# crabml/crabml

Measured on AMD Instinct MI355X. Metric: decode tokens/sec (batch-1 greedy), Llama-3-8B shape Q4_0, higher is better.
Workload: dtype q4_0 x q8_0 -> i32 dot, f32 accumulate

## Files before the change

### crabml_amd/csrc/fused.hip

```cpp
#include <chrono>
#include <thread>
#include <cmath>

#include "fused_common.hpp"
#include "fused_attention.hpp"
#include "fused_ffn.hpp"
#include "sampler.hpp"
#include "prefill_rows.hpp"
#include "lazy.hpp"


#include <dlfcn.h>

using namespace crabml_hip;

struct crabml_hip_tp_comm {
  crabml_hip_device* dev = nullptr;
  void* nccl = nullptr;
  int nranks = 1, rank = 0;
  bool p2p = false;
  bool connected = false;
  unsigned long long* inbox = nullptr;
  bool via_ipc[8] = {false};
  size_t inbox_bytes = 0;
  unsigned cap = 0;
  bool finegrained = false;
  void* peer[8] = {nullptr};
  int* fault = nullptr;
  unsigned host_epoch = 0;
  unsigned sessions = 0;
};
namespace {
struct NcclId {
  char b[128];
};
struct Rccl {
  typedef NcclId IdT;
  void* lib = nullptr;
  int (*GetUniqueId)(void*) = nullptr;
// ... 81 lines not shown
  float* h = nullptr;
  float* logits = nullptr;
  float* host_logits = nullptr;
  unsigned out_seq = 0;
  unsigned lazy_serial = 0;
  bool ext_kv = false;
  const crabml_hip_buf* ext_kc0 = nullptr;
  float* tmp = nullptr;
  char* act_dim = nullptr;
  char* act_attn = nullptr;
  char* act_hid = nullptr;
  float* rope = nullptr;
  int* state = nullptr;
  unsigned long long* slots = nullptr;
  unsigned long long* a8gran = nullptr;
  unsigned long long* h8gran = nullptr;
  bool q8k_producers = false;
  unsigned tp_salt = 0;
  bool tp_dry = false;
  bool k_norm_in = false;
  bool kfused = false;
  bool generic = false;
  bool ord = false;
  uint32_t qt = 0, out_qt = 0;
  float* xn = nullptr;
  bool norm_epi = false;
  bool defer_norm = false;
  float* rsums = nullptr;
  bool norm_epi_k = false;
  unsigned* out_tokens = nullptr;
  int out_cap = 0;
  float* am_val = nullptr;
  int* am_idx = nullptr;
  bool split_vocab = false;
  int vocab_l = 0, vocab_off = 0;
  int* am_best = nullptr;
  bool sampling = false;
  float* sm_bmax = nullptr;
  unsigned short* sm_keys = nullptr;
  unsigned* sm_hist = nullptr;
  float* sm_par = nullptr;
  float* sm_coins = nullptr;
  hipGraph_t sgraph[3] = {nullptr, nullptr, nullptr};
  hipGraphExec_t sexec[3] = {nullptr, nullptr, nullptr};
  size_t kv_len = 0;
  hipGraph_t graph[3] = {nullptr, nullptr, nullptr};
  hipGraphExec_t exec[3] = {nullptr, nullptr, nullptr};
  bool use_graph = false;
  bool capturing = false;
  int attn_variant = 0;
  size_t flash_ticket_until = 0;
  bool attn_long_ok = false;
  bool exact_long_ok = false;
  size_t attn_long_from = 0;
  bool pv_split = false;
  bool attn_flash = false;
  bool flash_ticket = false;
  bool attn_flash_rows = false;
  int flash_S = 0;
  int flash_min_rows = FLASH_MIN_ROWS;
  float* flash_part = nullptr;
  unsigned* flash_tick = nullptr;
  int gu_rows = 0;
  int attn_s_rows = 0;
  size_t attn_s_lds = 0;
  float* scores_g = nullptr;
// ... 299 lines not shown
  if (prof) prof_begin(dev, &ar, CRABML_HIP_F32, 7, 0.0);
  if (c->attn_s_rows > 0)
    launch_k(st, AR, attn_s_kernel(hd), dim3(n_heads + spare), dim3(256), c->attn_s_lds, (const float*)c->qbuf, (const unsigned short*)c->kc[l],
             (const unsigned short*)c->vc[l], pos_d, (const unsigned short*)dev->exp_table, c->attn, xq, xd, xisum, n_heads, n_kv, hd, seq_cap,
             c->attn_s_rows, pf, (k8 ? 2 : c->qt == CRABML_HIP_Q8_1 ? 1 : 0) | sbit, (long long*)nullptr, k8 ? *k8 : AttnQ8K{});
  else
    with_const_else<0, 1>(c->cfg.use_f16_kv_cache != 0, [&](auto kv16) {
      launch_k(st, AR, k_attn<decltype(kv16)::value != 0>, dim3(n_heads + spare), dim3(256), attn_lds, (const float*)c->qbuf, (const void*)c->kc[l],
               (const void*)c->vc[l], pos_d, (const unsigned short*)dev->exp_table, c->attn, xq, xd, xisum, n_heads, n_kv, hd,
               seq_cap, pf, (c->qt == CRABML_HIP_Q8_1 ? 1 : 0) | sbit, (long long*)nullptr);
    });
  if (prof) prof_end(dev, &ar);
}

int enqueue_classifier_and_sampler(crabml_hip_llama* c, const void* cls_act, bool prof) {
  crabml_hip_device* dev = c->dev;
  hipStream_t st = dev->stream;
  const auto& g = c->cfg;
  const int dim = (int)g.embedding_dim;
  int *token_d = c->state, *pos_d = c->state + 1, *step_d = c->state + 2;
  float* out = c->logits + c->vocab_off;
  crabml_hip_device::ProfRec pr{};
  const uint32_t ot = c->output->dtype;
  if (prof)
    CH_TRY(prof_begin(dev, &pr, ot, 5, (double)c->vocab_l * (double)(dim / block_elems(ot)) * (double)block_bytes(ot) + 4.0 * dim + 4.0 * c->vocab_l));
  if (dev->strict_order)
    CH_TRY(launch_gemv_strict(dev, c->output, (size_t)c->vocab_l, dim, cls_act, 1, out));
  else
    CH_TRY(launch_gemv(dev, c->output, (size_t)c->vocab_l, dim, cls_act, 1, out, prof ? &pr : nullptr));
  if (prof) CH_TRY(prof_end(dev, &pr));
  if (c->ext_kv) {
    if (c->host_logits != nullptr) {
      const int n = c->vocab_l;
      k_logits_to_host<<<64, 256, 0, st>>>((const f32x4*)out, (f32x4*)c->host_logits, n / 4, out, c->host_logits, n);
      k_host_flag<<<1, 1, 0, st>>>((unsigned*)(c->host_logits + c->cfg.vocab_size), (const int*)(c->state + 7), c->state + 5);
    }
    CH_HIP(dev, hipGetLastError());
    return 0;
  }
  if (c->sampling) {
    const int n = c->vocab_l;
    const SampleStep ss{c->sm_par, c->sm_coins, token_d, pos_d, step_d, c->state + 4, c->out_tokens, c->out_cap, c->state + 5};
    k_sample_max<<<SAMPLE_BLOCKS, 256, 0, st>>>(out, n, c->sm_par, c->sm_bmax);
    k_sample_keys<<<SAMPLE_BLOCKS, 256, 0, st>>>(out, n, c->sm_par, c->sm_bmax, SAMPLE_BLOCKS, (const unsigned short*)dev->exp_table,
                                                 c->sm_keys, c->sm_hist);
    if (dev->strict_order)
      k_sample_pick<true><<<1, SAMPLE_PICK_THREADS, 0, st>>>(c->sm_keys, n, c->sm_hist, ss);
    else
      k_sample_pick<false><<<1, SAMPLE_PICK_THREADS, 0, st>>>(c->sm_keys, n, c->sm_hist, ss);
    CH_HIP(dev, hipGetLastError());
    return 0;
  }
  k_argmax_partial<<<ARGMAX_BLOCKS, 256, 0, st>>>(out, c->vocab_l, c->am_val, c->am_idx, c->vocab_off);
  if (c->split_vocab && c->comm && c->comm->p2p)
    k_argmax_step_tp<<<1, 64, 0, st>>>(c->am_val, c->am_idx, ARGMAX_BLOCKS, token_d, pos_d, step_d, c->out_tokens, c->out_cap, c->state + 4,
                                       tp_view(c, true), n_segments(c));
  else
    k_argmax_step<<<1, 64, 0, st>>>(c->am_val, c->am_idx, ARGMAX_BLOCKS, token_d, pos_d, step_d, c->out_tokens, c->out_cap, c->state + 4,
                                    c->split_vocab ? c->am_best : (int*)nullptr);
  CH_HIP(dev, hipGetLastError());
  return 0;
}

static QkvEpiB qwen2_epi(const crabml_hip_llama* c, const QkvEpi& e, int l) {
  return QkvEpiB{e, (const float*)c->bq[l]->ptr, (const float*)c->bk[l]->ptr, (const float*)c->bv[l]->ptr};
}
template <class E>
struct QkvArchOf {
  static constexpr int value = QKV_LLAMA;
};
template <>
struct QkvArchOf<QkvEpiB> {
  static constexpr int value = QKV_QWEN2;
};
template <>
struct QkvArchOf<QkvEpiN> {
  static constexpr int value = QKV_GEMMA;
};
template <class F>
void with_qkv_epi(const crabml_hip_llama* c, const QkvEpi& e, int l, F&& f) {
  if (c->qwen2)
    f(qwen2_epi(c, e, l));
  else if (c->gemma)
    f(QkvEpiN{e});
  else
    f(e);
}
// ... 26 lines not shown
  const int L = (int)g.n_layers;
  constexpr bool Q81 = FMT == CRABML_HIP_Q4_1;
  const uint32_t qt = c->qt;
  ActPtrs ad = act_ptrs(c->act_dim, dim, qt), aa = act_ptrs(c->act_attn, dim_l, qt), ah = act_ptrs(c->act_hid, hidden_l, qt);
  const bool prof = dev->prof_on && !c->use_graph && !c->capturing;
  const double blk_b = (double)block_bytes(c->wtype) / 32.0;
  auto P0 = [&](crabml_hip_device::ProfRec* r, uint32_t stage, double rows, double k) {
    return prof ? prof_begin(dev, r, c->wtype, stage, rows * k * blk_b + 4.0 * k + 4.0 * rows) : 0;
  };
  auto P1 = [&](crabml_hip_device::ProfRec* r) { return prof ? prof_end(dev, r) : 0; };
  crabml_hip_device::ProfRec pr{};
  crabml_hip_device::ProfRec* R = prof ? &pr : nullptr;
  const bool do_pf = !(g.flags & CRABML_HIP_LLAMA_NO_PREFETCH);
  auto plan = [&](const crabml_hip_buf* a, const crabml_hip_buf* b, const crabml_hip_buf* cc) {
    PrefetchPlan pf{};
    const crabml_hip_buf* v[3] = {a, b, cc};
    for (int i = 0; i < 3; i++) {
      pf.p[i] = do_pf && v[i] ? v[i]->ptr : nullptr;
      pf.n[i] = do_pf && v[i] ? (v[i]->wl.total / 16) * 16 : 0;
    }
    pf.sink = c->state + 3;
    return pf;
  };
  const int spare = do_pf ? (dev->n_cu > 1 ? dev->n_cu - 1 : 0) : 0;
  const size_t norm_lds = norm_lds_bytes(dim);
  auto norm_quant = [&](const float* wn, float eps, bool add_pending, const PrefetchPlan& pf) {
    crabml_hip_device::ProfRec nr{};
    if (prof) prof_begin(dev, &nr, CRABML_HIP_F32, 6, 8.0 * dim);
    const float* addv = add_pending ? c->partial : nullptr;
    with_const_else<4, 12>(norm_nit(dim), [&](auto nit) {
      launch_k(st, prof ? &nr : nullptr, k_norm_quant<decltype(nit)::value, Q81>, dim3(1 + spare), dim3(1024), norm_lds, c->x, addv, wn, dim, eps, ad.q,
               ad.d, ad.isum, pf, c->ord ? 0 : 1);
    });
    if (prof) prof_end(dev, &nr);
  };
  const bool norm_epi = c->norm_epi;
  static const int qkv_upfront = test_hook_off("CRABML_HIP_QKV_UPFRONT") ? 0 : 1;
  const bool defer_wo = c->defer_norm && !Q81;
  const bool defer_down = c->defer_norm && !Q81;
  auto gemv_out = [&](const crabml_hip_buf* w, const ActPtrs& a, int k, uint32_t stage, const float* wnext, float eps_next, bool defer = false,
                      const float* xin = nullptr) -> int {
    CH_TRY(P0(&pr, stage, dim, k));
    float* dst = tp ? c->partial : c->x;
    if (norm_epi) {
      NormGather ng{c->slots, c->slots + dim / 16, c->state + 4, c->state + 5, n_segments(c), seg, c->rsums};
      const int split = chunk_split(g.flags, k, dim, dev->n_cu);
      c->tap.note(seg / 2, stage == 2 ? CRABML_HIP_PLAN_SPLIT_WO : CRABML_HIP_PLAN_SPLIT_DOWN, split);
      const TpP2P tpv = tp_view(c, tp);
      auto nq = [&](auto form, size_t lds, const float* rhs, auto tparg) {
        with_const_else<2, 1>(split, [&](auto s) {
          launch_k(st, R, nq_kernel<FMT, decltype(s)::value>(form), dim3(dim / 32 * split), dim3(1024), lds, planes_of(w), act_view<FMT>(a), rhs, c->x,
                   wnext, eps_next, ad.q, ad.d, ad.isum, ng, k / 32, Planes6{nullptr, 0}, tparg);
        });
      };
      if (xin != nullptr && !Q81) {
        if constexpr (!Q81) {
          if (tpv.n > 1)
            nq(NqForm<1, true>{}, q8_0_lds_bytes(k / 32), xin, tpv);
          else
            nq(NqForm<1>{}, q8_0_lds_bytes(k / 32), xin, NoTp{});
        }
      } else if (tpv.n > 1) {
        nq(NqForm<0, true>{}, 0, nullptr, tpv);
      } else if (c->ord) {
        static const int pipe_mode = test_hook_int("CRABML_HIP_ORD_PIPE", -1);
        const int pipe = pipe_mode >= 0 ? pipe_mode : FMT == CRABML_HIP_Q8_0 ? 2 : 1;
// ... 12 lines not shown
    } else if (c->ord) {
      launch_k(st, R, k_gemv_res_ord<FMT>, dim3((dim + 7) / 8), dim3(256), ord_terms_lds_bytes(k / 32), planes_of(w), act_view<FMT>(a), c->x, dim, k / 32);
    } else if (tp) {
      launch_k(st, R, k_gemv_res<FMT, 1, false>, dim3((dim + 1) / 2), dim3(128), 0, planes_of(w), act_view<FMT>(a), dst, dim, k / 32);
    } else {
      launch_k(st, R, k_gemv_res<FMT, 1, true>, dim3((dim + 1) / 2), dim3(128), 0, planes_of(w), act_view<FMT>(a), dst, dim, k / 32);
    }
    CH_TRY(P1(&pr));
    return 0;
  };

  const size_t ad_bytes = act_layout(qt, (size_t)dim).total, rs_bytes = c->rsums ? (size_t)(dim / 32) * 4 : 0;
  TapRec& tap = c->tap;
  auto TAP = [&](bool on, int f, const void* src, size_t bytes) -> int { return on ? tap.copy(c, f, src, bytes) : 0; };
  if (seg == 2 * L) {
    const void* cls_act = c->act_dim;
    if (c->out_qt != qt) {
      const float* addv = tp && !norm_epi ? c->partial : nullptr;
      launch_norm_f32(st, c->x, addv, (const float*)c->rms_final->ptr, dim, g.rms_norm_eps, c->xn, c->ord ? 0 : 1);
      if (c->out_qt == CRABML_HIP_F32) {
        cls_act = c->xn;
      } else {
        launch_quantize_act(st, c->out_qt, c->xn, (size_t)dim, c->act_dim);
      }
    } else if (!norm_epi) {
      norm_quant((const float*)c->rms_final->ptr, g.rms_norm_eps, tp, plan(nullptr, nullptr, nullptr));
      CH_TRY(TAP(tap.layer == L - 1, CRABML_HIP_TAP_DOWN_ACT, c->act_dim, ad_bytes));
    }
    CH_TRY(TAP(true, CRABML_HIP_TAP_CLS_ACT, cls_act, c->out_qt == CRABML_HIP_F32 ? (size_t)dim * 4 : act_layout(c->out_qt, (size_t)dim).total));
    return enqueue_classifier_and_sampler(c, cls_act, prof);
  }
  const int l = seg / 2;
  if ((seg & 1) == 0) {
    if (l == 0) launch_embed(c);
    if (!norm_epi || l == 0)
      norm_quant((const float*)c->rms_att[l]->ptr, g.rms_norm_eps, tp && l > 0, plan(c->wq[l], c->wk[l], c->wv[l]));
    const bool tl = tap.layer == l;
    if (!norm_epi || l == 0) tap.note(l, CRABML_HIP_PLAN_NORM_NIT, norm_nit(dim));
    CH_TRY(TAP(!norm_epi && l > 0 && tap.layer == l - 1, CRABML_HIP_TAP_DOWN_ACT, c->act_dim, ad_bytes));
    CH_TRY(TAP(tl, CRABML_HIP_TAP_QKV_IN_X, c->x, (size_t)dim * 4));
    CH_TRY(TAP(tl, CRABML_HIP_TAP_QKV_IN_ACT, c->act_dim, ad_bytes));
    CH_TRY(TAP(tl, CRABML_HIP_TAP_QKV_IN_RSUMS, c->rsums, rs_bytes));
    const QkvEpi e = decode_qkv_epi(c, l);
    const int total_rows = dim_l + 2 * kv_dim_l;
    CH_TRY(P0(&pr, 1, total_rows, dim));
    const RmsTail rtq{c->rsums, dim / 32, 1.0f / (float)dim, g.rms_norm_eps};
    const bool deferq = defer_down && l > 0;
    const int upfront = deferq ? qkv_upfront : (qkv_upfront && total_rows / 2 <= 4 * dev->n_cu) ? 1 : 0;
    if (!c->ord) {
      const int nu = dim / 32 * BlockFmt<FMT>::UNITS;
      tap.note(l, CRABML_HIP_PLAN_QKV_LOADER, deferq ? (upfront && nu == 128 ? 4 : 3) : (upfront && nu % 128 == 0 ? 2 : 1));
    }
    with_qkv_epi(c, e, l, [&](auto ep) {
      constexpr int A = QkvArchOf<decltype(ep)>::value;
      if (c->ord)
        launch_k(st, R, k_qkv_ord<FMT, A>, dim3((total_rows / 2 + 3) / 4), dim3(256), ord_terms_lds_bytes(dim / 32), planes_of(c->wq[l]),
                 planes_of(c->wk[l]), planes_of(c->wv[l]), act_view<FMT>(ad), dim / 32, ep, Planes6{nullptr, 0});
      else if (deferq) {
        if constexpr (!Q81)
          launch_k(st, R, k_qkv<FMT, true, A>, dim3((total_rows / 2 + 1) / 2), dim3(128), 0, planes_of(c->wq[l]), planes_of(c->wk[l]),
                   planes_of(c->wv[l]), act_view<FMT>(ad), dim / 32, ep, Planes6{nullptr, 0}, rtq, upfront);
      } else
        launch_k(st, R, k_qkv<FMT, false, A>, dim3((total_rows / 2 + 1) / 2), dim3(128), 0, planes_of(c->wq[l]), planes_of(c->wk[l]),
                 planes_of(c->wv[l]), act_view<FMT>(ad), dim / 32, ep, Planes6{nullptr, 0}, rtq, upfront);
    });
    CH_TRY(P1(&pr));
    CH_TRY(TAP(tl, CRABML_HIP_TAP_QBUF, c->qbuf, (size_t)dim_l * 4));
    const bool attn_quant = (hd % 32) == 0;
    const int attn_spare = do_pf && dev->n_cu > n_heads_l ? dev->n_cu - n_heads_l : 0;
// ... 255 lines not shown
         : c->wtype == CRABML_HIP_Q8_0 ? enqueue_segment_t<CRABML_HIP_Q8_0>(c, seg)
                                       : enqueue_segment_t<CRABML_HIP_Q4_1>(c, seg);
}

TpP2P p2p_view(const crabml_hip_tp_comm* m) {
  TpP2P t{};
  if (m && m->p2p) {
    for (int i = 0; i < 8; i++) t.peer[i] = (unsigned long long*)m->peer[i];
    t.n = m->nranks;
    t.me = m->rank;
    t.cap = m->cap;
    t.fault = m->fault;
  }
  return t;
}

int allreduce(crabml_hip_llama* c, int seg) {
  crabml_hip_device* dev = c->dev;
  if (c->tp_dry) return 0;
  if (c->comm && c->comm->p2p) {
    if (c->norm_epi) return 0;
    const int n = (int)c->cfg.embedding_dim;
    k_tp_allreduce<<<(n + 255) / 256, 256, 0, dev->stream>>>(c->partial, n, tp_view(c, true), c->state + 4, n_segments(c), seg, 0u, 0);
    CH_HIP(dev, hipGetLastError());
    return 0;
  }
  Rccl* r = rccl();
  if (!r || !c->comm || !c->comm->nccl) CH_BAIL(dev, CRABML_HIP_UNEXPECTED, "llama tp: no RCCL communicator");
  int rc = r->AllReduce(c->partial, c->partial, c->cfg.embedding_dim,  7,  0, c->comm->nccl, dev->stream);
  if (rc != 0) CH_BAIL(dev, CRABML_HIP_UNEXPECTED, "ncclAllReduce failed: %s", r->GetErrorString ? r->GetErrorString(rc) : "?");
  return 0;
}

int enqueue_step(crabml_hip_llama* c) {
  const int n = n_segments(c);
  for (int s = 0; s < n; s++) {
    CH_TRY(enqueue_segment(c, s));
    if (c->tp > 1 && s + 1 < n) CH_TRY(allreduce(c, s));
  }
  return 0;
}

int run_step(crabml_hip_llama* c, size_t pos) {
  const int variant = variant_of(c, pos);
  if (c->use_graph && c->exec[variant]) {
    CH_HIP(c->dev, hipGraphLaunch(c->exec[variant], c->dev->stream));
    return 0;
  }
  c->attn_variant = variant;
  return enqueue_step(c);
}

int run_step_sampled(crabml_hip_llama* c, size_t pos) {
  const int variant = variant_of(c, pos);
  crabml_hip_device* dev = c->dev;
  int rc = 0;
  c->sampling = true;
  if (c->use_graph && !c->sexec[variant]) {
    hipError_t e = hipStreamBeginCapture(dev->stream, hipStreamCaptureModeThreadLocal);
    if (e != hipSuccess) {
      c->sampling = false;
      return hip_fail(dev, e, "llama: sampler graph capture", __FILE__, __LINE__);
    }
    c->capturing = true;
    c->attn_variant = variant;
    const int erc = enqueue_step(c);
    c->capturing = false;
    hipGraph_t graph = nullptr;
    e = hipStreamEndCapture(dev->stream, &graph);
    hipGraphExec_t exec = nullptr;
    if (erc == 0 && e == hipSuccess && graph && hipGraphInstantiate(&exec, graph, nullptr, nullptr, 0) == hipSuccess) {
      c->sgraph[variant] = graph;
      c->sexec[variant] = exec;
    } else {
      if (graph) (void)hipGraphDestroy(graph);
      (void)hipGetLastError();
      c->sampling = false;
      CH_BAIL(dev, CRABML_HIP_UNEXPECTED, "llama: hipGraph capture/instantiate of the sampled step failed");
// ... 1009 lines not shown
          const FlashFn tfn = flash_kernel((int)grp, (int)hd, qt == CRABML_HIP_Q8_1, true);
          if (until > 0 && tfn != nullptr && raise_dyn_lds(dev, (const void*)tfn, (int)flash_lds_bytes((int)grp, (int)hd)) == hipSuccess)
            c->flash_ticket_until = until;
          (void)hipGetLastError();
        }
        if (c->attn_flash && flash_rows_kernel((int)hd) != nullptr &&
            raise_dyn_lds(dev, (const void*)flash_rows_kernel((int)hd), (int)flash_rows_lds_bytes((int)hd)) == hipSuccess)
          c->attn_flash_rows = true;
        (void)hipGetLastError();
        if (c->attn_flash && g.attn_long_from == 0) c->attn_long_from = 96;
      }
      (void)hipGetLastError();
    }
    if (g.use_f16_kv_cache && hd % 8 == 0 && !(g.flags & CRABML_HIP_LLAMA_NO_STAGED_ATTENTION)) {
      const size_t S = c->attn_long_ok && c->attn_long_from < g.seq_len ? c->attn_long_from : g.seq_len;
      const size_t lds = attn_s_lds_bytes((int)S, (int)hd);
      if (lds <= 150 * 1024 && raise_dyn_lds(dev, (const void*)attn_s_kernel((int)hd), (int)lds) == hipSuccess) {
        c->attn_s_rows = (int)S;
        c->attn_s_lds = lds;
      }
      (void)hipGetLastError();
    }
  }
  A(8 * sizeof(int), (void**)&c->state);
  A((g.embedding_dim / 16 + g.embedding_dim) * 8, (void**)&c->slots);
  const bool p2p_comm = c->comm != nullptr && c->comm->p2p;
  c->norm_epi = !generic && !c->kfused && (tp == 1 || p2p_comm || c->tp_dry) && !(g.flags & CRABML_HIP_LLAMA_NO_NORM_EPILOGUE) &&
                (int)(g.embedding_dim / 32) <= dev->n_cu;
  c->norm_epi_k = c->kfused && wt == CRABML_HIP_Q4_K && out_qt == CRABML_HIP_Q8_K && tp == 1 &&
                  !(g.flags & CRABML_HIP_LLAMA_NO_NORM_EPILOGUE) && g.embedding_dim % 256 == 0 && (int)(g.embedding_dim / 32) <= dev->n_cu;
  c->defer_norm = c->norm_epi && tp == 1 && !ord && !dev->strict_order && (wt == CRABML_HIP_Q4_0 || wt == CRABML_HIP_Q8_0) &&
                  !(g.flags & CRABML_HIP_LLAMA_EXACT_NORM) && (int)(g.embedding_dim / 32) <= dev->n_cu;
  if (c->defer_norm) A(g.embedding_dim / 16 * 4, (void**)&c->rsums);
  if (c->norm_epi && tp > 1 && !ord && !dev->strict_order && (wt == CRABML_HIP_Q4_0 || wt == CRABML_HIP_Q8_0) &&
      !(g.flags & CRABML_HIP_LLAMA_NO_H_CONSUMER_QUANT) && hidden_l % 32 == 0 && (int)(hidden_l / 32) * 2 <= dev->n_cu && !dry) {
    int pick = 0;
    for (int r = 30; r >= 2 && !pick; r -= 2)
      if (hidden_l % r == 0 && (int)(hidden_l / r) >= dev->n_cu && (int)(hidden_l / r) <= 2 * dev->n_cu) pick = r;
    if (pick && q8_0_lds_bytes((int)(hidden_l / 32)) <= 60 * 1024) c->gu_rows = pick;
  }
  c->q8k_producers = c->norm_epi_k && !(g.flags & (CRABML_HIP_LLAMA_NO_RHS_PROLOGUE | CRABML_HIP_LLAMA_NO_Q8K_PRODUCERS)) && dim_l % 256 == 0 &&
                     hidden_l % 256 == 0 && (hd == 64 || hd == 128 || hd == 256) && (int)(hidden_l / 32) <= 2 * dev->n_cu;
  c->k_norm_in = c->q8k_producers && wt == CRABML_HIP_Q4_K && tp == 1 && !ord && !dev->strict_order && g.embedding_dim % 256 == 0 && g.embedding_dim / 256 <= 32 &&
                 !(g.flags & (CRABML_HIP_LLAMA_NO_K_NORM_IN | CRABML_HIP_LLAMA_SPLIT_CHUNKS_ALWAYS | CRABML_HIP_LLAMA_SPLIT_CHUNKS_NEVER));
  if (c->k_norm_in && !c->rsums) A(g.embedding_dim / 16 * 4, (void**)&c->rsums);
  if (c->q8k_producers) {
    A(dim_l * 8, (void**)&c->a8gran);
    A(hidden_l * 8, (void**)&c->h8gran);
  }
  c->out_cap = (int)g.seq_len;
  A((size_t)c->out_cap * 4, (void**)&c->out_tokens);
  A(ARGMAX_BLOCKS * 4, (void**)&c->am_val);
  A(ARGMAX_BLOCKS * 4, (void**)&c->am_idx);
  A(2 * sizeof(int), (void**)&c->am_best);
  if (rc != 0) {
    crabml_hip_llama_destroy(c);
    return rc;
  }
  {
    std::vector<float> tab(g.seq_len * (size_t)(c->npairs ? c->npairs : 1) * 2, 0.f);
    const float theta_scale = powf(10000.0f, -2.0f / (float)hd);
    for (size_t p = 0; p < g.seq_len; p++) {
      if (qwen2 || gemma) {
        rope_table_neox(tab.data() + p * c->npairs * 2, p, hd, (size_t)c->npairs);
        continue;
      }
      float theta = (float)p;
      for (int i = 0; i < c->npairs; i++) {
        tab[(p * c->npairs + i) * 2] = cosf(theta);
        tab[(p * c->npairs + i) * 2 + 1] = sinf(theta);
        theta *= theta_scale;
      }
    }
    hipError_t e = dry ? hipErrorUnknown : hipMemcpyAsync(c->rope, tab.data(), tab.size() * 4, hipMemcpyHostToDevice, dev->stream);
    if (dry) {
      *out = c;
      return 0;
    }
    if (e == hipSuccess) e = hipMemsetAsync(c->state, 0, 8 * sizeof(int), dev->stream);
    if (e == hipSuccess && c->split_vocab) e = hipMemsetD32Async((hipDeviceptr_t)c->logits, (int)0xff800000u, g.vocab_size, dev->stream);
    if (e == hipSuccess) e = hipMemsetAsync(c->slots, 0, (g.embedding_dim / 16 + g.embedding_dim) * 8, dev->stream);
    if (e == hipSuccess && c->a8gran) e = hipMemsetAsync(c->a8gran, 0, dim_l * 8, dev->stream);
    if (e == hipSuccess && c->h8gran) e = hipMemsetAsync(c->h8gran, 0, hidden_l * 8, dev->stream);
    if (e == hipSuccess) e = hipStreamSynchronize(dev->stream);
    if (e != hipSuccess) {
      crabml_hip_llama_destroy(c);
      return hip_fail(dev, e, "llama init", __FILE__, __LINE__);
    }
  }
  const bool want_graph = !(g.flags & CRABML_HIP_LLAMA_NO_GRAPH) &&
                          (tp == 1 || c->tp_dry || p2p_comm || (c->comm != nullptr && (g.flags & CRABML_HIP_LLAMA_TP_GRAPH)));
  if (want_graph) {
    const int nvar = c->attn_long_ok ? (c->flash_ticket_until > 0 ? 3 : 2) : 1;
    bool ok = true;
    for (int v = 0; v < nvar && ok; v++) {
      ok = false;
      hipError_t e = hipStreamBeginCapture(dev->stream, hipStreamCaptureModeThreadLocal);
      if (e != hipSuccess) break;
      c->capturing = true;
      c->attn_variant = v;
      int erc = enqueue_step(c);
      c->capturing = false;
      hipGraph_t graph = nullptr;
      hipError_t e2 = hipStreamEndCapture(dev->stream, &graph);
      if (erc == 0 && e2 == hipSuccess && graph) {
        hipGraphExec_t exec = nullptr;
        if (hipGraphInstantiate(&exec, graph, nullptr, nullptr, 0) == hipSuccess) {
          c->graph[v] = graph;
          c->exec[v] = exec;
          ok = true;
        } else {
          (void)hipGraphDestroy(graph);
        }
      } else if (graph) {
        (void)hipGraphDestroy(graph);
      }
    }
    (void)hipGetLastError();
    c->use_graph = ok;
    c->attn_variant = 0;
    if (!ok && tp == 1) {
      crabml_hip_llama_destroy(c);
      CH_BAIL(dev, CRABML_HIP_UNEXPECTED, "llama: hipGraph capture/instantiate failed");
    }
  }
  *out = c;
  return 0;
}

extern "C" {

int crabml_hip_llama_create(crabml_hip_device_t* dev, const crabml_hip_llama_config_t* cfg,
                            const crabml_hip_llama_weights_t* w, crabml_hip_llama_t** out) {
  if (!dev || !cfg || !w || !out) return CRABML_HIP_BAD_INPUT;
  *out = nullptr;
  CH_LIVE(dev);
  CH_USE(dev);
  CH_FLUSH(dev);
  return llama_create_impl(dev, cfg, w, nullptr, nullptr, out);
}

int crabml_hip_llama_create_arch(crabml_hip_device_t* dev, const crabml_hip_llama_config_t* cfg, const crabml_hip_llama_weights_t* w,
                                 const crabml_hip_llama_arch_t* arch, crabml_hip_llama_t** out) {
// ... 470 lines not shown
  const size_t L = m.cfg.n_layers;
  if (m.rms_att.size() != L || m.rms_ffn.size() != L || m.wq.size() != L || m.wk.size() != L || m.wv.size() != L || m.wo.size() != L ||
      m.gate.size() != L || m.down.size() != L || m.up.size() != L || m.kc.size() != L || m.vc.size() != L)
    return CRABML_HIP_BAD_INPUT;
  if (m.arch == CRABML_HIP_ARCH_LLAMA) return llama_create_impl(dev, &m.cfg, &w, m.kc.data(), m.vc.data(), out);
  if (m.arch == CRABML_HIP_ARCH_GEMMA) {
    const crabml_hip_llama_arch_t arch{CRABML_HIP_ARCH_GEMMA, nullptr, nullptr, nullptr};
    return llama_create_impl(dev, &m.cfg, &w, m.kc.data(), m.vc.data(), out, &arch);
  }
  if (m.bq.size() != L || m.bk.size() != L || m.bv.size() != L) return CRABML_HIP_BAD_INPUT;
  const crabml_hip_llama_arch_t arch{CRABML_HIP_ARCH_QWEN2, m.bq.data(), m.bk.data(), m.bv.data()};
  return llama_create_impl(dev, &m.cfg, &w, m.kc.data(), m.vc.data(), out, &arch);
}

void lazy_ctx_destroy(crabml_hip_llama* c) { (void)crabml_hip_llama_destroy(c); }

bool lazy_ctx_orphaned(const crabml_hip_llama* c) {
  auto sole = [&](const crabml_hip_buf* b) {
    if (!b) return false;
    int holds = 0;
    for (const crabml_hip_buf* h : c->held)
      if (h == b) holds++;
    return holds > 0 && b->refcnt.load() <= holds;
  };
  return sole(c->wq.empty() ? nullptr : c->wq[0]) || (c->qwen2 && sole(c->bq[0])) || (c->ext_kv && sole(c->ext_kc0));
}

int lazy_ctx_n_segments(const crabml_hip_llama* c) { return n_segments(c); }

int lazy_ctx_begin(crabml_hip_llama* c, size_t token, size_t pos) {
  if (c->dev->dry) return 0;
  c->lazy_serial += 2;
  c->out_seq++;
  k_set_state5<<<1, 1, 0, c->dev->stream>>>(c->state, (int)token, (int)pos, 0, (int)c->lazy_serial, (int)c->out_seq);
  CH_HIP(c->dev, hipGetLastError());
  c->attn_variant = variant_of(c, pos);
  c->kv_len = pos + 1;
  return 0;
}

int lazy_ctx_segment(crabml_hip_llama* c, int seg) {
  if (c->dev->dry) return 0;
  return enqueue_segment(c, seg);
}

bool lazy_ctx_has_graph(const crabml_hip_llama* c) { return !c->dev->dry && c->use_graph && c->exec[0] != nullptr; }
int lazy_ctx_step(crabml_hip_llama* c, size_t pos) {
  if (c->dev->dry) return 0;
  return run_step(c, pos);
}

int lazy_ctx_copy_logits(crabml_hip_llama* c, float* dst) {
  if (c->dev->dry) return 0;
  CH_HIP(c->dev, hipMemcpyAsync(dst, c->logits, c->cfg.vocab_size * 4, hipMemcpyDeviceToDevice, c->dev->stream));
  return 0;
}

int lazy_ctx_final_norm(crabml_hip_llama* c, float* dst) {
  crabml_hip_device* dev = c->dev;
  if (dev->dry) return 0;
  const int dim = (int)c->cfg.embedding_dim;
  const int half = dev->strict_order ? 0 : 1;
  launch_norm_f32(dev->stream, c->x, nullptr, (const float*)c->rms_final->ptr, dim, c->cfg.rms_norm_eps, dst, half);
  CH_HIP(dev, hipGetLastError());
  return 0;
}

int lazy_ctx_fault_request(crabml_hip_llama* c) {
// ... 31 lines not shown
```

### crabml_amd/csrc/fused_attention.hpp

```cpp
#pragma once
#include "fused_common.hpp"

namespace crabml_hip {
template <bool KV16, bool STAMP = false>
__global__ __launch_bounds__(256) void k_attn(const float* __restrict__ q, const void* __restrict__ kc,
                                              const void* __restrict__ vc, const int* __restrict__ pos_d,
                                              const unsigned short* __restrict__ exp_tab, float* __restrict__ out,
                                              signed char* __restrict__ xq, unsigned short* __restrict__ xd,
                                              void* __restrict__ xisum, int n_heads, int n_kv, int hd, int seq_cap,
                                              PrefetchPlan pf, int q81_in, long long* __restrict__ stamps = nullptr) {
  const int q81 = q81_in & 255;
  const bool strict_sum = (q81_in & 256) != 0;
  if ((int)blockIdx.x >= n_heads) {
    prefetch_wg(pf, blockIdx.x - n_heads, gridDim.x - n_heads);
    return;
  }
  auto stamp = [&](int i) {
    if constexpr (STAMP) {
      if (blockIdx.x == 0 && blockIdx.y == 0 && threadIdx.x == 0) stamps[i] = (long long)__builtin_readcyclecounter();
    }
  };
  stamp(0);
  extern __shared__ float lds[];
  __shared__ float s_red[4];
// ... 244 lines not shown
        kv[i] = *(const i32x4*)(kr + 8 * i);
        qq[i] = *(const i32x4*)(q16 + 8 * i);
      }
#pragma unroll
      for (int i = 0; i < 16; i++) {
#pragma unroll
        for (int j = 0; j < 4; j++) {
          const h2q kh = __builtin_bit_cast(h2q, (unsigned)kv[i][j]), qh = __builtin_bit_cast(h2q, (unsigned)qq[i][j]);
          acc = __builtin_fmaf((float)qh[0], (float)kh[0], acc);
          acc = __builtin_fmaf((float)qh[1], (float)kh[1], acc);
        }
      }
    } else {
      for (int i = 0; i < hd; i += 8) {
        const i32x4 kv = *(const i32x4*)(kr + i), qq = *(const i32x4*)(q16 + i);
#pragma unroll
        for (int j = 0; j < 4; j++) {
          const h2q kh = __builtin_bit_cast(h2q, (unsigned)kv[j]), qh = __builtin_bit_cast(h2q, (unsigned)qq[j]);
          acc = __builtin_fmaf((float)qh[0], (float)kh[0], acc);
          acc = __builtin_fmaf((float)qh[1], (float)kh[1], acc);
        }
      }
    }
    return acc;
  };
  if (seq <= 64) {
    if (wave == 0) {
      const float sc = lane < seq ? score_of(lane) : -INFINITY;
      stamp(2);
      const float mx = wave_max_f32(sc);
      const float e = lane < seq ? exp_cached_f(sc - mx, exp_tab) : 0.0f;
      float sum = 0.0f;
#pragma unroll
      for (int i = 0; i < 64; i++) sum += rl_f(e, i);
      const float pv = e / sum;
      if (lane < seq) scores[lane] = h2f(f2h(pv));
    }
    __syncthreads();
  } else {
    for (int t = tid; t < seq; t += 256) scores[t] = score_of(t);
    __syncthreads();
    stamp(2);
    softmax_row<true>(scores, seq, exp_tab, s_red, &s_val, strict_sum);
  }
  stamp(3);
  typedef _Float16 h2v __attribute__((ext_vector_type(2)));
  const int npair = hd >> 1;
  float v0 = 0.0f, v1 = 0.0f;
  if (tid < npair) {
    const unsigned* vr = (const unsigned*)Vs + tid;
    h2v c = {(_Float16)0.0f, (_Float16)0.0f};
    int t = 0;
    for (; t + 8 <= seq; t += 8) {
      unsigned vv[8];
      float pp[8];
#pragma unroll
      for (int u = 0; u < 8; u++) {
        vv[u] = vr[(size_t)(t + u) * npair];
        pp[u] = scores[t + u];
      }
#pragma unroll
      for (int u = 0; u < 8; u++) {
        const _Float16 ph = (_Float16)pp[u];
        const h2v p2 = {ph, ph};
        const h2v prod = __builtin_bit_cast(h2v, vv[u]) * p2;
        c = c + prod;
      }
// ... 1155 lines not shown
```

### include/crabml_hip_debug.h

```cpp
#ifndef CRABML_HIP_DEBUG_H
#define CRABML_HIP_DEBUG_H

#include "crabml_hip.h"

#ifdef __cplusplus
extern "C" {
#endif

#define CRABML_HIP_FLAG_LAZY_NO_FUSION 4
#define CRABML_HIP_FLAG_DRY 0x40000000
int crabml_hip_debug_lazy_stats(crabml_hip_device_t* dev, uint64_t* out, size_t cap);

int crabml_hip_debug_device_numa_node(crabml_hip_device_t* dev, int32_t* node);

int crabml_hip_debug_quantize(crabml_hip_device_t* dev, const crabml_hip_buf_t* x, size_t n, uint32_t qtype,
                              void* dst, size_t dst_bytes);
int crabml_hip_debug_block_dots(crabml_hip_device_t* dev, const crabml_hip_buf_t* w, size_t m, size_t k, size_t row,
                                const crabml_hip_buf_t* x, int32_t* dst);
int crabml_hip_debug_superblock_ints(crabml_hip_device_t* dev, const crabml_hip_buf_t* w, size_t m, size_t k, size_t row,
                                     const crabml_hip_buf_t* x, int32_t variant, int32_t* dst, float* value);
int crabml_hip_debug_gemm_ints(crabml_hip_device_t* dev, const crabml_hip_buf_t* w, size_t m, size_t k,
                               const crabml_hip_buf_t* x, size_t b, int32_t* dst, float* out);
int crabml_hip_debug_gemm_f16w(crabml_hip_device_t* dev, const crabml_hip_buf_t* const* w, const size_t* m, size_t nw, size_t k,
                               const crabml_hip_buf_t* x, size_t b, int32_t rows_path, uint16_t junk, const int32_t* force,
                               float* const* out, uint16_t* xh, int32_t* used, void* hq, uint16_t* hxh);
int crabml_hip_debug_read_ceiling(crabml_hip_device_t* dev, size_t bytes, int32_t reps, double* gbytes_per_s);

int crabml_hip_debug_flash_attention(crabml_hip_device_t* dev, const float* q, const uint16_t* k, const uint16_t* v, size_t n_heads,
                                     size_t n_kv, size_t head_dim, size_t seq, size_t slices, float* out, float* out2);

int crabml_hip_debug_flash_attention_rows(crabml_hip_device_t* dev, const float* q, const uint16_t* k, const uint16_t* v, size_t n_heads,
                                          size_t n_kv, size_t head_dim, size_t pos0, size_t rows, size_t seq_cap, float* out);

int crabml_hip_debug_sample(crabml_hip_device_t* dev, const float* logits, size_t n, float temperature, float topp, float coin,
                            uint32_t* token);

#define CRABML_HIP_LLAMA_NO_NORM_EPILOGUE 4
#define CRABML_HIP_LLAMA_NO_KQUANT_FUSION 256
#define CRABML_HIP_LLAMA_Q4_1_SEGMENTS 512
#define CRABML_HIP_LLAMA_NO_TILE_ATTENTION 2048
#define CRABML_HIP_LLAMA_NO_RHS_PROLOGUE 1024
#define CRABML_HIP_LLAMA_TP_DRY_RUN 128
#define CRABML_HIP_LLAMA_NO_LONG_ATTENTION 64
#define CRABML_HIP_LLAMA_NO_Q8K_PRODUCERS 32768
#define CRABML_HIP_LLAMA_Q8K_ATTN_PRODUCER 65536
#define CRABML_HIP_LLAMA_NO_PV_PRODUCER_WAVES 131072
#define CRABML_HIP_LLAMA_NO_PREFILL_ROW_FUSION 262144
#define CRABML_HIP_LLAMA_NO_PV_ROW_TILES 16384
#define CRABML_HIP_LLAMA_NO_STAGED_ATTENTION 8192
#define CRABML_HIP_LLAMA_FLASH_TICKET 2097152
#define CRABML_HIP_LLAMA_NO_H_CONSUMER_QUANT 4096
#define CRABML_HIP_LLAMA_PREFILL_INT8_GEMM 524288
#define CRABML_HIP_LLAMA_PREFILL_SEPARATE_F16_ROWS 33554432
#define CRABML_HIP_LLAMA_PREFILL_NO_GU_EPILOGUE 67108864
#define CRABML_HIP_LLAMA_NO_K_NORM_IN 16777216
#define CRABML_HIP_LLAMA_SPLIT_CHUNKS_ALWAYS 16
#define CRABML_HIP_LLAMA_SPLIT_CHUNKS_NEVER 32

int crabml_hip_llama_debug_kv(crabml_hip_llama_t* ctx, size_t layer, int32_t which_v, void* dst, size_t nbytes);

enum {
  CRABML_HIP_TAP_QKV_IN_X = 0,
  CRABML_HIP_TAP_QKV_IN_ACT = 1,
  CRABML_HIP_TAP_QKV_IN_RSUMS = 2,
  CRABML_HIP_TAP_QBUF = 3,
  CRABML_HIP_TAP_ATTN = 4,
  CRABML_HIP_TAP_ACT_ATTN = 5,
  CRABML_HIP_TAP_WO_X = 6,
  CRABML_HIP_TAP_WO_ACT = 7,
  CRABML_HIP_TAP_WO_RSUMS = 8,
  CRABML_HIP_TAP_ACT_HID = 9,
  CRABML_HIP_TAP_DOWN_X = 10,
  CRABML_HIP_TAP_DOWN_ACT = 11,
  CRABML_HIP_TAP_DOWN_RSUMS = 12,
  CRABML_HIP_TAP_CLS_ACT = 13,
  CRABML_HIP_TAP_PLAN = 14,
  CRABML_HIP_TAP_FIELDS = 15
};
enum {
  CRABML_HIP_PLAN_N_CU = 0,
  CRABML_HIP_PLAN_DEFER_NORM = 1,
  CRABML_HIP_PLAN_NORM_EPILOGUE = 2,
  CRABML_HIP_PLAN_ATTN_VARIANT = 3,
  CRABML_HIP_PLAN_SPLIT_WO = 4,
  CRABML_HIP_PLAN_SPLIT_DOWN = 5,
  CRABML_HIP_PLAN_QKV_LOADER = 6,
  CRABML_HIP_PLAN_NORM_NIT = 7,
  CRABML_HIP_TAP_PLAN_WORDS = 8
// ... 87 lines not shown
```

Baseline: 685.6.

## Fold token-boundary kernels: embed+norm, argmax ticket, logits export flag, state via args

Fuses the first-layer embedding lookup into the norm-quantize kernel and merges the argmax partial and step kernels into one using a last-block ticket. The logits-export and host-flag kernels are merged the same way. Per-token state is passed as kernel arguments, patched into the captured graph's root node, instead of a separate set-state launch. It also lets the attention softmax sum skip lanes past the sequence length. These changes cut several tiny launches per decode step, at the cost of atomic ticket counters and graph-node parameter updates.

```diff
diff --git a/crabml_amd/csrc/fused.hip b/crabml_amd/csrc/fused.hip
--- a/crabml_amd/csrc/fused.hip
+++ b/crabml_amd/csrc/fused.hip
@@ -5,6 +5,7 @@
 #include "fused_common.hpp"
 #include "fused_attention.hpp"
 #include "fused_ffn.hpp"
+#include "token_ends.hpp"
 #include "sampler.hpp"
 #include "prefill_rows.hpp"
 #include "lazy.hpp"
@@ -152,6 +153,31 @@
   int out_cap = 0;
   float* am_val = nullptr;
   int* am_idx = nullptr;
+  bool fold_head = false, fold_export = false, fold_argmax = false;
+  unsigned* end_tick = nullptr;
+  struct HeadArgs {
+    const char* ew;
+    int dtype;
+    size_t off_scale;
+    int* st;
+    HeadState hs;
+    float scale;
+    float* x;
+    const float* w;
+    int cols;
+    float eps;
+    signed char* q;
+    unsigned short* d;
+    void* isum;
+    PrefetchPlan pf;
+    int half;
+    void* ptrs[15];
+    hipKernelNodeParams params;
+  };
+  bool state_by_args = false;
+  HeadState head_state{-1, 0, 0, 0, 0};
+  HeadArgs head_args[3] = {};
+  hipGraphNode_t head_node[3] = {nullptr, nullptr, nullptr};
   bool split_vocab = false;
   int vocab_l = 0, vocab_off = 0;
   int* am_best = nullptr;
@@ -517,8 +543,14 @@
   if (c->ext_kv) {
     if (c->host_logits != nullptr) {
       const int n = c->vocab_l;
-      k_logits_to_host<<<64, 256, 0, st>>>((const f32x4*)out, (f32x4*)c->host_logits, n / 4, out, c->host_logits, n);
-      k_host_flag<<<1, 1, 0, st>>>((unsigned*)(c->host_logits + c->cfg.vocab_size), (const int*)(c->state + 7), c->state + 5);
+      unsigned* flag = (unsigned*)(c->host_logits + c->cfg.vocab_size);
+      if (c->fold_export) {
+        k_logits_to_host_flag<<<64, 256, 0, st>>>((const f32x4*)out, (f32x4*)c->host_logits, n / 4, out, c->host_logits, n, c->end_tick, flag,
+                                                  (const int*)(c->state + 7), c->state + 5);
+      } else {
+        k_logits_to_host<<<64, 256, 0, st>>>((const f32x4*)out, (f32x4*)c->host_logits, n / 4, out, c->host_logits, n);
+        k_host_flag<<<1, 1, 0, st>>>(flag, (const int*)(c->state + 7), c->state + 5);
+      }
     }
     CH_HIP(dev, hipGetLastError());
     return 0;
@@ -536,8 +568,15 @@
     CH_HIP(dev, hipGetLastError());
     return 0;
   }
+  const bool p2p_vocab = c->split_vocab && c->comm && c->comm->p2p;
+  if (c->fold_argmax && !p2p_vocab) {
+    k_argmax_ticket_step<<<ARGMAX_BLOCKS, 256, 0, st>>>(out, c->vocab_l, c->am_val, c->am_idx, c->vocab_off, c->end_tick + 1, token_d, pos_d, step_d,
+                                                        c->out_tokens, c->out_cap, c->state + 4, c->split_vocab ? c->am_best : (int*)nullptr);
+    CH_HIP(dev, hipGetLastError());
+    return 0;
+  }
   k_argmax_partial<<<ARGMAX_BLOCKS, 256, 0, st>>>(out, c->vocab_l, c->am_val, c->am_idx, c->vocab_off);
-  if (c->split_vocab && c->comm && c->comm->p2p)
+  if (p2p_vocab)
     k_argmax_step_tp<<<1, 64, 0, st>>>(c->am_val, c->am_idx, ARGMAX_BLOCKS, token_d, pos_d, step_d, c->out_tokens, c->out_cap, c->state + 4,
                                        tp_view(c, true), n_segments(c));
   else
@@ -630,6 +669,19 @@
       launch_k(st, prof ? &nr : nullptr, k_norm_quant<decltype(nit)::value, Q81>, dim3(1 + spare), dim3(1024), norm_lds, c->x, addv, wn, dim, eps, ad.q,
                ad.d, ad.isum, pf, c->ord ? 0 : 1);
     });
+    if (prof) prof_end(dev, &nr);
+  };
+  auto embed_norm_quant = [&](const float* wn, float eps, const PrefetchPlan& pf) {
+    crabml_hip_device::ProfRec nr{};
+    if (prof) prof_begin(dev, &nr, CRABML_HIP_F32, 6, 8.0 * dim);
+    const HeadState hs = c->state_by_args && !c->capturing ? c->head_state : HeadState{-1, 0, 0, 0, 0};
+    crabml_hip_llama::HeadArgs a{(const char*)c->token_embed->ptr, (int)c->token_embed->dtype, c->token_embed->wl.off_scale, c->state, hs, c->embed_scale,
+                                 c->x, wn, dim, eps, ad.q, ad.d, ad.isum, pf, c->ord ? 0 : 1, {}, {}};
+    with_const_else<4, 12>(norm_nit(dim), [&](auto nit) {
+      launch_k(st, prof ? &nr : nullptr, k_embed_norm_quant<decltype(nit)::value, Q81>, dim3(1 + spare), dim3(1024), norm_lds, a.ew, a.dtype, a.off_scale,
+               a.st, a.hs, a.scale, a.x, a.w, a.cols, a.eps, a.q, a.d, a.isum, a.pf, a.half);
+    });
+    if (c->capturing) c->head_args[c->attn_variant] = a;
     if (prof) prof_end(dev, &nr);
   };
   const bool norm_epi = c->norm_epi;
@@ -708,9 +760,13 @@
   }
   const int l = seg / 2;
   if ((seg & 1) == 0) {
-    if (l == 0) launch_embed(c);
-    if (!norm_epi || l == 0)
-      norm_quant((const float*)c->rms_att[l]->ptr, g.rms_norm_eps, tp && l > 0, plan(c->wq[l], c->wk[l], c->wv[l]));
+    if (l == 0 && c->fold_head) {
+      embed_norm_quant((const float*)c->rms_att[l]->ptr, g.rms_norm_eps, plan(c->wq[l], c->wk[l], c->wv[l]));
+    } else {
+      if (l == 0) launch_embed(c);
+      if (!norm_epi || l == 0)
+        norm_quant((const float*)c->rms_att[l]->ptr, g.rms_norm_eps, tp && l > 0, plan(c->wq[l], c->wk[l], c->wv[l]));
+    }
     const bool tl = tap.layer == l;
     if (!norm_epi || l == 0) tap.note(l, CRABML_HIP_PLAN_NORM_NIT, norm_nit(dim));
     CH_TRY(TAP(!norm_epi && l > 0 && tap.layer == l - 1, CRABML_HIP_TAP_DOWN_ACT, c->act_dim, ad_bytes));
@@ -1032,6 +1088,23 @@
   return 0;
 }
 
+bool bind_head_node(crabml_hip_llama* c, int v) {
+  size_t n = 0;
+  if (hipGraphGetRootNodes(c->graph[v], nullptr, &n) != hipSuccess || n != 1) return false;
+  hipGraphNode_t node = nullptr;
+  hipGraphNodeType type;
+  if (hipGraphGetRootNodes(c->graph[v], &node, &n) != hipSuccess || hipGraphNodeGetType(node, &type) != hipSuccess || type != hipGraphNodeTypeKernel)
+    return false;
+  crabml_hip_llama::HeadArgs& a = c->head_args[v];
+  if (hipGraphKernelNodeGetParams(node, &a.params) != hipSuccess || a.params.blockDim.x != 1024 || a.st != c->state) return false;
+  void* ptrs[15] = {&a.ew, &a.dtype, &a.off_scale, &a.st, &a.hs, &a.scale, &a.x, &a.w, &a.cols, &a.eps, &a.q, &a.d, &a.isum, &a.pf, &a.half};
+  for (int i = 0; i < 15; i++) a.ptrs[i] = ptrs[i];
+  a.params.kernelParams = a.ptrs;
+  a.params.extra = nullptr;
+  c->head_node[v] = node;
+  return true;
+}
+
 int enqueue_step(crabml_hip_llama* c) {
   const int n = n_segments(c);
   for (int s = 0; s < n; s++) {
@@ -1044,6 +1117,10 @@
 int run_step(crabml_hip_llama* c, size_t pos) {
   const int variant = variant_of(c, pos);
   if (c->use_graph && c->exec[variant]) {
+    if (c->state_by_args) {
+      c->head_args[variant].hs = c->head_state;
+      CH_HIP(c->dev, hipGraphExecKernelNodeSetParams(c->exec[variant], c->head_node[variant], &c->head_args[variant].params));
+    }
     CH_HIP(c->dev, hipGraphLaunch(c->exec[variant], c->dev->stream));
     return 0;
   }
@@ -2119,6 +2196,16 @@
   c->defer_norm = c->norm_epi && tp == 1 && !ord && !dev->strict_order && (wt == CRABML_HIP_Q4_0 || wt == CRABML_HIP_Q8_0) &&
                   !(g.flags & CRABML_HIP_LLAMA_EXACT_NORM) && (int)(g.embedding_dim / 32) <= dev->n_cu;
   if (c->defer_norm) A(g.embedding_dim / 16 * 4, (void**)&c->rsums);
+  {
+    const int sep_hook = test_hook_int("CRABML_HIP_SEPARATE_TOKEN_ENDS", 0);
+    const bool sep_head = (g.flags & CRABML_HIP_LLAMA_SEPARATE_HEAD) || (sep_hook & 1);
+    const bool sep_export = (g.flags & CRABML_HIP_LLAMA_SEPARATE_LOGITS_EXPORT) || (sep_hook & 2);
+    const bool sep_argmax = (g.flags & CRABML_HIP_LLAMA_SEPARATE_ARGMAX) || (sep_hook & 4);
+    c->fold_head = !sep_head && !generic && !c->kfused && tp == 1;
+    c->fold_export = !sep_export;
+    c->state_by_args = c->fold_head && ext_kc != nullptr && !((g.flags & CRABML_HIP_LLAMA_SEPARATE_STATE) || (sep_hook & 8));
+    c->fold_argmax = !sep_argmax;
+  }
   if (c->norm_epi && tp > 1 && !ord && !dev->strict_order && (wt == CRABML_HIP_Q4_0 || wt == CRABML_HIP_Q8_0) &&
       !(g.flags & CRABML_HIP_LLAMA_NO_H_CONSUMER_QUANT) && hidden_l % 32 == 0 && (int)(hidden_l / 32) * 2 <= dev->n_cu && !dry) {
     int pick = 0;
@@ -2140,6 +2227,7 @@
   A(ARGMAX_BLOCKS * 4, (void**)&c->am_val);
   A(ARGMAX_BLOCKS * 4, (void**)&c->am_idx);
   A(2 * sizeof(int), (void**)&c->am_best);
+  A(2 * sizeof(unsigned), (void**)&c->end_tick);
   if (rc != 0) {
     crabml_hip_llama_destroy(c);
     return rc;
@@ -2165,6 +2253,7 @@
       return 0;
     }
     if (e == hipSuccess) e = hipMemsetAsync(c->state, 0, 8 * sizeof(int), dev->stream);
+    if (e == hipSuccess) e = hipMemsetAsync(c->end_tick, 0, 2 * sizeof(unsigned), dev->stream);
     if (e == hipSuccess && c->split_vocab) e = hipMemsetD32Async((hipDeviceptr_t)c->logits, (int)0xff800000u, g.vocab_size, dev->stream);
     if (e == hipSuccess) e = hipMemsetAsync(c->slots, 0, (g.embedding_dim / 16 + g.embedding_dim) * 8, dev->stream);
     if (e == hipSuccess && c->a8gran) e = hipMemsetAsync(c->a8gran, 0, dim_l * 8, dev->stream);
@@ -2196,6 +2285,7 @@
           c->graph[v] = graph;
           c->exec[v] = exec;
           ok = true;
+          if (c->state_by_args && !bind_head_node(c, v)) c->state_by_args = false;
         } else {
           (void)hipGraphDestroy(graph);
         }
@@ -2732,8 +2822,12 @@
   if (c->dev->dry) return 0;
   c->lazy_serial += 2;
   c->out_seq++;
-  k_set_state5<<<1, 1, 0, c->dev->stream>>>(c->state, (int)token, (int)pos, 0, (int)c->lazy_serial, (int)c->out_seq);
-  CH_HIP(c->dev, hipGetLastError());
+  if (c->state_by_args) {
+    c->head_state = HeadState{(int)token, (int)pos, 0, (int)c->lazy_serial, (int)c->out_seq};
+  } else {
+    k_set_state5<<<1, 1, 0, c->dev->stream>>>(c->state, (int)token, (int)pos, 0, (int)c->lazy_serial, (int)c->out_seq);
+    CH_HIP(c->dev, hipGetLastError());
+  }
   c->attn_variant = variant_of(c, pos);
   c->kv_len = pos + 1;
   return 0;
diff --git a/crabml_amd/csrc/fused_attention.hpp b/crabml_amd/csrc/fused_attention.hpp
--- a/crabml_amd/csrc/fused_attention.hpp
+++ b/crabml_amd/csrc/fused_attention.hpp
@@ -300,7 +300,11 @@
       const float e = lane < seq ? exp_cached_f(sc - mx, exp_tab) : 0.0f;
       float sum = 0.0f;
 #pragma unroll
-      for (int i = 0; i < 64; i++) sum += rl_f(e, i);
+      for (int b = 0; b < 64; b += 8) {
+        if (b >= seq) break;
+#pragma unroll
+        for (int i = 0; i < 8; i++) sum += rl_f(e, b + i);
+      }
       const float pv = e / sum;
       if (lane < seq) scores[lane] = h2f(f2h(pv));
     }
diff --git a/crabml_amd/csrc/token_ends.hpp b/crabml_amd/csrc/token_ends.hpp
--- /dev/null
+++ b/crabml_amd/csrc/token_ends.hpp
@@ -0,0 +1,133 @@
+#pragma once
+#include "fused_common.hpp"
+#include "fused_ffn.hpp"
+
+namespace crabml_hip {
+
+struct HeadState {
+  int token, pos, step, serial, out_seq;
+};
+template <int NIT, bool Q81>
+__global__ __launch_bounds__(1024) void k_embed_norm_quant(const char* __restrict__ ew, int dtype, size_t off_scale, int* __restrict__ st, HeadState hs,
+                                                          float scale, float* __restrict__ x, const float* __restrict__ w, int cols, float eps,
+                                                          signed char* __restrict__ q, unsigned short* __restrict__ d, void* __restrict__ isum,
+                                                          PrefetchPlan pf, int half) {
+  if (blockIdx.x > 0) {
+    prefetch_wg(pf, blockIdx.x - 1, gridDim.x - 1);
+    return;
+  }
+  extern __shared__ float lds[];
+  __shared__ float s_rms;
+  NormLds L{lds, lds + cols};
+  int token;
+  if (hs.token >= 0) {
+    if (threadIdx.x == 0) {
+      st[0] = hs.token;
+      st[1] = hs.pos;
+      st[2] = hs.step;
+      st[4] = hs.serial;
+      st[7] = hs.out_seq;
+    }
+    token = hs.token;
+  } else {
+    token = st[0];
+  }
+  const size_t row = (size_t)token * cols;
+#pragma unroll
+  for (int it = 0; it < NIT; it++) {
+    const int i = it * 1024 + threadIdx.x;
+    if (i < cols) {
+      const float v = dequant_elem(ew, dtype, off_scale, row + i);
+      if (scale != 1.0f)
+        x[i] = v * scale;
+      else
+        x[i] = v;
+    }
+  }
+  norm_quant_block<NIT, true, Q81>(x, nullptr, w, cols, eps, L, &s_rms, q, d, isum, nullptr, half);
+}
+
+__device__ __forceinline__ bool last_ticket(unsigned* tick) {
+  asm volatile("s_waitcnt vmcnt(0)" ::: "memory");
+  const unsigned t = __hip_atomic_fetch_add(tick, 1u, __ATOMIC_RELAXED, __HIP_MEMORY_SCOPE_AGENT);
+  if (t != gridDim.x - 1) return false;
+  __hip_atomic_store(tick, 0u, __ATOMIC_RELAXED, __HIP_MEMORY_SCOPE_AGENT);
+  return true;
+}
+
+__global__ __launch_bounds__(256) void k_logits_to_host_flag(const f32x4* __restrict__ src, f32x4* __restrict__ dst, int n4,
+                                                             const float* __restrict__ src1, float* __restrict__ dst1, int n,
+                                                             unsigned* __restrict__ tick, unsigned* __restrict__ flag,
+                                                             const int* __restrict__ seq_d, const int* __restrict__ fault) {
+  for (int i = blockIdx.x * 256 + threadIdx.x; i < n4; i += gridDim.x * 256) __builtin_nontemporal_store(src[i], dst + i);
+  if (blockIdx.x == 0 && threadIdx.x < (n & 3)) dst1[n4 * 4 + threadIdx.x] = src1[n4 * 4 + threadIdx.x];
+  __threadfence_system();
+  __syncthreads();
+  if (threadIdx.x != 0 || !last_ticket(tick)) return;
+  __threadfence_system();
+  const unsigned seq = (unsigned)*seq_d;
+  flag[1] = (unsigned)*fault;
+  __threadfence_system();
+  __hip_atomic_store(flag, seq, __ATOMIC_RELEASE, __HIP_MEMORY_SCOPE_SYSTEM);
+}
+
+__global__ __launch_bounds__(256) void k_argmax_ticket_step(const float* __restrict__ logits, int n, float* __restrict__ pv, int* __restrict__ pi, int base,
+                                                            unsigned* __restrict__ tick, int* __restrict__ token_d, int* __restrict__ pos_d,
+                                                            int* __restrict__ step_d, unsigned* __restrict__ out_tokens, int out_cap,
+                                                            int* __restrict__ serial_d, int* __restrict__ best) {
+  __shared__ float sv[4];
+  __shared__ int si[4];
+  const int per = (n + gridDim.x - 1) / gridDim.x;
+  const int lo = blockIdx.x * per, hi = min(n, lo + per);
+  float bv = -INFINITY;
+  int bi = -1;
+  for (int i = lo + threadIdx.x; i < hi; i += blockDim.x) argmax_combine(bv, bi, logits[i], base + i);
+#pragma unroll
+  for (int o = 32; o > 0; o >>= 1) {
+    float ov = __shfl_xor(bv, o, 64);
+    int oi = __shfl_xor(bi, o, 64);
+    argmax_combine(bv, bi, ov, oi);
+  }
+  if ((threadIdx.x & 63) == 0) {
+    sv[threadIdx.x >> 6] = bv;
+    si[threadIdx.x >> 6] = bi;
+  }
+  __syncthreads();
+  if (threadIdx.x >= 64) return;
+  int last = 0;
+  if (threadIdx.x == 0) {
+    for (int w = 1; w < 4; w++) argmax_combine(bv, bi, sv[w], si[w]);
+    __hip_atomic_store(pv + blockIdx.x, bv, __ATOMIC_RELAXED, __HIP_MEMORY_SCOPE_AGENT);
+    __hip_atomic_store(pi + blockIdx.x, bi, __ATOMIC_RELAXED, __HIP_MEMORY_SCOPE_AGENT);
+    __builtin_amdgcn_fence(__ATOMIC_RELEASE, "agent");
+    last = last_ticket(tick) ? 1 : 0;
+  }
+  if (!__builtin_amdgcn_readfirstlane(last)) return;
+  __builtin_amdgcn_fence(__ATOMIC_ACQUIRE, "agent");
+  const int nparts = (int)gridDim.x;
+  bv = -INFINITY;
+  bi = -1;
+  for (int i = threadIdx.x; i < nparts; i += 64)
+    argmax_combine(bv, bi, __hip_atomic_load(pv + i, __ATOMIC_RELAXED, __HIP_MEMORY_SCOPE_AGENT),
+                   __hip_atomic_load(pi + i, __ATOMIC_RELAXED, __HIP_MEMORY_SCOPE_AGENT));
+#pragma unroll
+  for (int o = 32; o > 0; o >>= 1) {
+    float ov = __shfl_xor(bv, o, 64);
+    int oi = __shfl_xor(bi, o, 64);
+    argmax_combine(bv, bi, ov, oi);
+  }
+  if (threadIdx.x == 0) {
+    if (best != nullptr) {
+      best[0] = __builtin_bit_cast(int, bv);
+      best[1] = bi;
+    }
+    *token_d = bi;
+    int st = *step_d;
+    if (st < out_cap) out_tokens[st] = (unsigned)bi;
+    *step_d = st + 1;
+    *pos_d = *pos_d + 1;
+    *serial_d = *serial_d + 1;
+  }
+}
+
+}
diff --git a/include/crabml_hip_debug.h b/include/crabml_hip_debug.h
--- a/include/crabml_hip_debug.h
+++ b/include/crabml_hip_debug.h
@@ -54,6 +54,13 @@
 #define CRABML_HIP_LLAMA_PREFILL_SEPARATE_F16_ROWS 33554432
 #define CRABML_HIP_LLAMA_PREFILL_NO_GU_EPILOGUE 67108864
 #define CRABML_HIP_LLAMA_NO_K_NORM_IN 16777216
+#define CRABML_HIP_LLAMA_SEPARATE_HEAD 134217728
+#define CRABML_HIP_LLAMA_SEPARATE_LOGITS_EXPORT 268435456
+#define CRABML_HIP_LLAMA_SEPARATE_ARGMAX 536870912
+#define CRABML_HIP_LLAMA_SEPARATE_STATE 1073741824
+#define CRABML_HIP_LLAMA_SEPARATE_TOKEN_ENDS                                                                         \
+  (CRABML_HIP_LLAMA_SEPARATE_HEAD | CRABML_HIP_LLAMA_SEPARATE_LOGITS_EXPORT | CRABML_HIP_LLAMA_SEPARATE_ARGMAX | \
+   CRABML_HIP_LLAMA_SEPARATE_STATE)
 #define CRABML_HIP_LLAMA_SPLIT_CHUNKS_ALWAYS 16
 #define CRABML_HIP_LLAMA_SPLIT_CHUNKS_NEVER 32
 
```

New measurement: 685.7, median of 4. Within noise of the previous version (+0.0%).
